# bacpop/ska.rust

Hardware: AMD Instinct MI355X
Metric: genomes/sec ska build+align, 1 000x5 Mbp k=31; bit-exact vs CPU (higher is better)
Workload: dtype u64

## Files before the change

ska.rust_amd/csrc/skx_api.cpp:

```cpp
#include "skx_internal.h"
#include "../../include/skx_host.h"
#include <algorithm>
#include <atomic>
#include <chrono>
#include <cmath>
#include <cstdarg>
#include <cstddef>
#include <cstdio>
#include <cstring>
#include <map>
#include <memory>
#include <mutex>
#include <numeric>
#include <optional>
#include <unordered_map>
#include <thread>
#include <cerrno>
#include <fcntl.h>
#include <sys/mman.h>
#include <sys/stat.h>
#include <unistd.h>

using namespace skx;

// ... 670 lines not shown
                std::vector<skx_key> nk; nk.reserve(kept);
                for (uint64_t i = 0; i < U; i++) if (hkeep[i] == 1) nk.push_back(a->host_keys[i]);
                a->host_keys.swap(nk);
            }
            a->n_kmers = kept;
        }
        SKX_HIP(hipStreamSynchronize(st));
        a->matrix = std::move(nm); a->present = std::move(p2); a->unambig = std::move(u2); a->mask = std::move(m2); a->vcount = std::move(v2);
        a->pitch = np; a->n_rows = kept;
        a->drop_lazy();
        a->stats_ready = true;
    }
    return SKX_OK;
}

extern "C" int skx_array_filter(skx_array *a, uint64_t min_count, int filter_ambig_as_missing, int filter_type, int mask_ambig,
                                int ignore_const_gaps, int update_kmers, int32_t *removed)
{
    return skx_guarded([&]() -> int {
    skx_ctx *ctx = a->ctx; hipStream_t st = ctx->stream;
    SKX_HIP(hipSetDevice(ctx->device));
    const uint64_t U = a->n_rows; const size_t S = a->names.size();
    ctx->cut_ranks = ctx->cut_blocks = 0;
    DevBuf<unsigned long long> tally;
    unsigned long long h_tally[2] = {0, 0};
    if (a->pieces && !a->stats_ready && !filter_ambig_as_missing && min_count >= 2 && a->total_samples == 0 && !knob("stats_eager"))
        SKX_TRY(pieces_stats_pass(a, min_count, &tally));
    else
        SKX_TRY(array_lazy_stats(a));
    DevBuf<uint8_t> keep; DevBuf<uint64_t> pos;
    SKX_TRY(keep.alloc(U)); SKX_TRY(pos.alloc(U + 1));
    uint64_t kept = 0, silent = 0;
    {
        StageTimer t(ctx, &ctx->tm.filter);
        FilterArgs fa{a->vcount.p, a->present.p, a->unambig.p, a->mask.p, U, (uint32_t)(a->total_samples ? a->total_samples : S), min_count, filter_ambig_as_missing, filter_type, ignore_const_gaps, keep.p};
        launch_filter_flags(fa, st);
        DevBuf<uint32_t> sc_sums; DevBuf<uint64_t> sc_offs;
        SKX_TRY(sc_sums.alloc(scan_u8_blocks(U))); SKX_TRY(sc_offs.alloc(scan_u8_blocks(U) + 1));
        launch_scan_u8(keep.p, pos.p, U, sc_sums.p, sc_offs.p, st);
        SKX_HIP(hipMemcpyAsync(&kept, pos.p + U, 8, hipMemcpyDeviceToHost, st));
        if (tally.p) SKX_HIP(hipMemcpyAsync(h_tally, tally.p, 16, hipMemcpyDeviceToHost, st));
// ... 380 lines not shown
```

ska.rust_amd/csrc/skx_append.hip:

```cpp
#include "skx_device.h"
#include <cstdlib>
#include <type_traits>

namespace skx {

typedef uint32_t u32x4 __attribute__((ext_vector_type(4)));
typedef const u32x4 __attribute__((address_space(1))) *g4_t;

#ifdef SKX_AP_PROF
__device__ unsigned long long g_ap_prof[16];
#define AP_PROF_START unsigned long long tprof = __builtin_readcyclecounter(), tacc[12] = {0, 0, 0, 0, 0, 0, 0, 0, 0, 0, 0, 0}
#define AP_PROF(i) do { const unsigned long long t_ = __builtin_readcyclecounter(); tacc[(i)] += t_ - tprof; tprof = t_; } while (0)
#define AP_PROF_FLUSH() do { for (int i_ = 0; i_ < 12; i_++) if (tacc[i_] && (i_ >= 6 || (threadIdx.x & 63) == 0)) atomicAdd(&g_ap_prof[i_], tacc[i_]); } while (0)
extern "C" void skx_debug_phase_prof(unsigned long long *out, int reset)
{
    unsigned long long h[16];
    (void)hipDeviceSynchronize();
    (void)hipMemcpyFromSymbol(h, HIP_SYMBOL(g_ap_prof), sizeof(h));
    for (int i = 0; i < 16; i++) out[i] = h[i];
    if (reset) { for (auto &x : h) x = 0; (void)hipMemcpyToSymbol(HIP_SYMBOL(g_ap_prof), h, sizeof(h)); }
}
#else
#define AP_PROF_START do { } while (0)
#define AP_PROF(i) do { } while (0)
// ... 501 lines not shown
        uint32_t rc = min_count ? cut : 0xFFFFFFFFu;
        if (ncnt && ncnt[j] > stage) rc = 0xFFFFFFFFu;
        r_cut[j] = rc;
        if (tally && nrank) pieces_cut_tally(nrank[j], rc, tally);
    }
}
void launch_pieces_cut(const uint16_t *plen, int n_samples, uint32_t cap, uint32_t min_count, const uint32_t *nrank, const uint32_t *ncnt, uint32_t stage, int n_blocks,
                       uint32_t *r_cut, unsigned long long *tally, hipStream_t st)
{
    if (n_blocks <= 0) return;
    hipLaunchKernelGGL(pieces_cut_kernel, dim3((unsigned)n_blocks), dim3(256), ((size_t)cap + 1) * 4, st, plen, n_samples, cap, min_count, nrank, ncnt, stage, r_cut, tally);
}

__global__ __launch_bounds__(256) void pieces_stats_kernel(const uint8_t *pieces, const uint16_t *plen, const uint16_t *perm, const uint32_t *nrank, const uint32_t *ncnt,
                                                           const uint64_t *roff, uint32_t cap, int S, uint32_t *o_present, uint32_t *o_unambig, uint32_t *o_mask,
                                                           uint32_t *o_vcount, int force_direct, uint32_t stage, uint32_t min_count, unsigned long long *tally)
{
    constexpr int W = 4;
    extern __shared__ __attribute__((aligned(16))) uint16_t s_stage[];
    const uint32_t PS_STAGE = stage;
    uint16_t *const s_pr = s_stage, *const s_un = s_stage + stage, *const s_mk = s_stage + 2 * (size_t)stage;
    const uint64_t j = blockIdx.x;
    const uint32_t nr = nrank[j], nrows = ncnt[j];
    const uint64_t r0 = roff[j];
    if (blockIdx.y * 256u * 8u * W >= nr && !(blockIdx.y == 0 && nrows)) return;
    const bool staged = gridDim.y == 1 && nrows <= PS_STAGE && !force_direct;
    const int lane = threadIdx.x & 63, wv = __builtin_amdgcn_readfirstlane((int)(threadIdx.x >> 6));
    const uint16_t *pl = plen + j * (uint64_t)S;
    uint32_t lim = nr;
    if (min_count && staged) {
        const uint32_t rc = pieces_cut_block(pl, S, cap, min_count, reinterpret_cast<uint32_t *>(s_stage));
        if (threadIdx.x == 0 && tally) pieces_cut_tally(nr, rc, tally);
        if (rc < lim) lim = rc;
    }
    const uint32_t nseen = (lim + 31u) / 32u * 32u < nr ? (lim + 31u) / 32u * 32u : nr;
    const uint32_t ncol = (lim + 31u) / 32u, ncg = ncol < 64u ? ncol : 64u;
    uint32_t G = 4, P = 1;
    if (staged && ncol) {
        G = (ncol + 63u) / 64u;
        for (P = 4u / G; P > 1u && (P / 2u) * G * 36u * 4u * ncg > PS_STAGE * 6u; P >>= 1) { }
    }
// ... 133 lines not shown
            const uint32_t r = rb + (uint32_t)src, prow = (uint32_t)__shfl((int)pp, src, 64);
            uint32_t m = 0;
            for (int t = lane; t < S; t += 64) {
                if ((uint32_t)pl[t] <= r) continue;
                const uint32_t x = *(reinterpret_cast<const uint32_t *>(pieces + (j * (uint64_t)S + t) * (cap / 2)) + (r >> 3));
                const uint32_t nib = (x >> ((r & 7u) * 4u)) & 15u;
                if (nib) m |= 1u << nib;
            }
#pragma unroll
            for (int dd = 32; dd >= 1; dd >>= 1) m |= __shfl_xor(m, dd, 64);
            if (lane == 0) { if (staged) s_mk[prow] = (uint16_t)m; else o_mask[r0 + prow] = m; }
        }
    }
    if (!staged) return;
    __syncthreads();
    for (uint32_t p = threadIdx.x; p < nrows; p += 256) {
        const uint32_t pr = s_pr[p];
        o_present[r0 + p] = pr; o_vcount[r0 + p] = pr;
        o_unambig[r0 + p] = s_un[p]; o_mask[r0 + p] = s_mk[p];
    }
}
namespace {
struct StatsLaunch { unsigned gy; int direct; uint32_t stage; bool bounded() const { return gy == 1 && !direct; } };
StatsLaunch stats_launch(uint32_t cap)
{
    static const int direct = knob("stats_direct") ? 1 : 0;
    return {(cap / 32 + 255u) / 256u, direct, (cap + 63u) / 64u * 64u};
}
}
void launch_pieces_stats(const uint8_t *pieces, const uint16_t *plen, const uint16_t *perm, const uint32_t *nrank, const uint32_t *ncnt, const uint64_t *roff, uint32_t cap,
                         int n_samples, int n_blocks, uint32_t *present, uint32_t *unambig, uint32_t *mask, uint32_t *vcount, hipStream_t st, uint32_t min_count, unsigned long long *tally)
{
    if (n_blocks <= 0) return;
    const StatsLaunch l = stats_launch(cap);
    if (!l.bounded()) min_count = 0;
    hipLaunchKernelGGL(pieces_stats_kernel, dim3((unsigned)n_blocks, l.gy), dim3(256), (size_t)l.stage * 6, st, pieces, plen, perm, nrank, ncnt, roff, cap, n_samples, present, unambig, mask, vcount,
                       l.direct, l.stage, min_count, tally);
}
uint32_t pieces_stats_bound(uint32_t cap) { const StatsLaunch l = stats_launch(cap); return l.bounded() ? l.stage : 0u; }
__global__ __launch_bounds__(256) void pieces_cells_kernel(const uint8_t *pieces, const uint16_t *plen, uint32_t cap, int S, unsigned long long *out)
{
    const uint64_t j = blockIdx.x;
    const int lane = threadIdx.x & 63;
    for (int s = blockIdx.y * 4 + (threadIdx.x >> 6); s < S; s += gridDim.y * 4) {
        const uint32_t pl = plen[j * (uint64_t)S + s];
        const uint32_t *src = reinterpret_cast<const uint32_t *>(pieces + (j * (uint64_t)S + s) * (cap / 2));
        uint32_t c = 0;
        for (uint32_t i = lane; i < (pl + 7u) / 8u; i += 64) { const uint32_t x = src[i]; uint32_t t = x | (x >> 1); t |= t >> 2; c += (uint32_t)__popc(t & 0x11111111u); }
#pragma unroll
        for (int dd = 32; dd >= 1; dd >>= 1) c += __shfl_xor(c, dd, 64);
        if (lane == 0 && c) atomicAdd(&out[s], (unsigned long long)c);
    }
// ... 29 lines not shown
    const uint32_t hi = __builtin_amdgcn_perm(0x4E42444Bu, 0x56535247u, idx);
    const uint32_t sel = ((m >> 3) & 0x01010101u) * 0xFFu;
    return (hi & sel) | (lo & ~sel);
}
template <bool KEPT>
__global__ __launch_bounds__(64 * PR_WAVES) void pieces_rows_kernel(PiecesRowsArgs a)
{
    extern __shared__ __attribute__((aligned(16))) unsigned char s_raw[];
    const uint32_t cap = a.cap;
    uint16_t *s_src = reinterpret_cast<uint16_t *>(s_raw);
    uint32_t *s_piece = reinterpret_cast<uint32_t *>(s_raw + (((size_t)cap + 16) * 2 + 15) / 16 * 16);
    const uint64_t j = (uint64_t)blockIdx.x + a.j_base;
    const uint32_t n = a.ncnt[j];
    if (n == 0) return;
    const uint64_t r0 = a.roff[j];
    const uint64_t k0 = KEPT ? a.kpos[r0] : 0;
    const uint32_t nout = KEPT ? (uint32_t)(a.kpos[r0 + n] - k0) : n;
    if (nout == 0) return;
    const int tid = threadIdx.x, lane = tid & 63, wv = tid >> 6;
    const uint64_t ocol = KEPT ? k0 : r0 - a.col_base;
    const uint32_t shift = (uint32_t)(ocol & 3u);
    const uint32_t ndw = (nout + shift + 3u) / 4u;
    const uint16_t *pj = a.perm + j * (uint64_t)cap;
    const uint32_t nr = a.nrank[j];
    const int S = a.n_samples;
    const int s_lo = blockIdx.y * a.samples_per_wg, s_hi = s_lo + a.samples_per_wg < S ? s_lo + a.samples_per_wg : S;
    uint32_t *pc = s_piece + (size_t)wv * (cap / 8 + 4);
    const unsigned char *pcb = reinterpret_cast<const unsigned char *>(pc);
    __shared__ uint32_t s_top;
    uint32_t nrw = (nr + 7u) / 8u;
    if (lane < 4) pc[cap / 8 + lane] = 0u;
    for (uint32_t t0 = 0; t0 < nout + shift; t0 += cap) {
        for (uint32_t i = tid; i < cap + 16u; i += blockDim.x) s_src[i] = (uint16_t)cap;
        if (KEPT && tid == 0) s_top = 0;
        __syncthreads();
        uint32_t top = 0;
        for (uint32_t r = tid; r < nr; r += blockDim.x) {
            const uint32_t p = pj[r];
            if (p == 0xFFFFu || p >= n) continue;
            uint32_t sc;
            if (!KEPT) sc = shift + p;
            else if (a.keep[r0 + p] == 1) sc = shift + (uint32_t)(a.kpos[r0 + p] - k0);
            else continue;
            if (sc >= t0 && sc < t0 + cap) { s_src[sc - t0] = (uint16_t)r; top = r + 1u; }
        }
        if (KEPT && top) atomicMax(&s_top, top);
        __syncthreads();
        if (KEPT && !a.full_pieces) nrw = (s_top + 7u) / 8u;
        const uint32_t v_lo = t0 / 4u, v_hi = (t0 + cap) / 4u < ndw ? (t0 + cap) / 4u : ndw;
        const int cnt = __builtin_amdgcn_readfirstlane(s_lo + wv < s_hi ? (s_hi - s_lo - wv + PR_WAVES - 1) / PR_WAVES : 0);
        const uint32_t n4 = (nrw + 3u) / 4u;
        const uint16_t *plj = a.plen + j * (uint64_t)S + s_lo + wv;
        uint4 *pc4 = reinterpret_cast<uint4 *>(pc);
        auto masked = [&](uint4 x, uint32_t i, uint32_t plw) {
            if (4u * i >= plw) x.x = 0u;
            if (4u * i + 1u >= plw) x.y = 0u;
// ... 46 lines not shown
            }
            __builtin_amdgcn_wave_barrier();
        }
        __syncthreads();
    }
}
void launch_pieces_rows(const PiecesRowsArgs &a, uint32_t n_blocks, hipStream_t st)
{
    if (!n_blocks || a.n_samples <= 0) return;
    PiecesRowsArgs b = a;
    int spw = a.n_samples;
    while (spw > PR_WAVES * 4 && (uint64_t)n_blocks * ((a.n_samples + spw - 1) / spw) < 8192) spw = (spw + 1) / 2;
    b.samples_per_wg = spw;
    const unsigned gy = (unsigned)((a.n_samples + spw - 1) / spw);
    const size_t lds = (((size_t)a.cap + 16) * 2 + 15) / 16 * 16 + (size_t)PR_WAVES * (a.cap / 8 + 4) * 4;
    if (a.keep) {
        (void)hipFuncSetAttribute((const void *)pieces_rows_kernel<true>, hipFuncAttributeMaxDynamicSharedMemorySize, (int)lds);
        hipLaunchKernelGGL(pieces_rows_kernel<true>, dim3(n_blocks, gy), dim3(64 * PR_WAVES), lds, st, b);
    } else {
        (void)hipFuncSetAttribute((const void *)pieces_rows_kernel<false>, hipFuncAttributeMaxDynamicSharedMemorySize, (int)lds);
        hipLaunchKernelGGL(pieces_rows_kernel<false>, dim3(n_blocks, gy), dim3(64 * PR_WAVES), lds, st, b);
    }
}

}

#include "skx_append_wide.inc"
```

ska.rust_amd/csrc/skx_device.h:

```cpp
#pragma once
#include <hip/hip_runtime.h>
#include <stdint.h>

namespace skx {

long knob(const char *name, long absent = 0);
int extract_tile_bases(int logB);
constexpr int MAX_LOGB = 13;
constexpr uint64_t EMPTY64 = ~0ull;

struct HashParams {
    int bits;
    int hb;
    uint32_t hmask;
    uint32_t c[4];
};
HashParams make_hash_params(int k);
__host__ __device__ inline uint32_t hround(uint32_t v, uint32_t c, int hb) { return (v * c) >> (32 - hb); }
__host__ __device__ inline void hmix_halves(uint32_t &L, uint32_t &R, const HashParams &p)
{
    L ^= hround(R, p.c[0], p.hb); R ^= hround(L, p.c[1], p.hb);
}
__host__ __device__ inline uint64_t hmix(uint64_t x, const HashParams &p)
{
// ... 120 lines not shown
    uint32_t nslots, cap;
    uint8_t *pieces; uint16_t *plen; uint16_t *perm; uint32_t *nrank;
    uint64_t *stage; uint32_t stride; uint32_t *ncnt;
    unsigned long long *probe;
    int *overflow;
    uint32_t rounds = 1;
    int *bar = nullptr;
};
bool append_ok(int bits, int logB, int logQ, uint32_t region_cap, uint32_t nslots, uint32_t cap);
void launch_append(const AppendArgs &a, uint32_t region_cap, hipStream_t st);
void launch_append_probe(const AppendArgs &a, uint32_t region_cap, unsigned blocks, hipStream_t st);
constexpr uint32_t APPEND_WIDE_MAX_CAP = 3072, APPEND_WIDE_MAX_SLOTS = 4096;
bool append_wide_ok(int bits, int logB, int logQ, uint32_t nslots, uint32_t cap);
void launch_append_wide(const AppendArgs &a, hipStream_t st);
void launch_append_wide_probe(const AppendArgs &a, unsigned blocks, hipStream_t st);
void launch_pieces_stats(const uint8_t *pieces, const uint16_t *plen, const uint16_t *perm, const uint32_t *nrank, const uint32_t *ncnt, const uint64_t *roff, uint32_t cap,
                         int n_samples, int n_blocks, uint32_t *present, uint32_t *unambig, uint32_t *mask, uint32_t *vcount, hipStream_t st, uint32_t min_count = 0, unsigned long long *tally = nullptr);
void launch_pieces_cut(const uint16_t *plen, int n_samples, uint32_t cap, uint32_t min_count, const uint32_t *nrank, const uint32_t *ncnt, uint32_t stage, int n_blocks,
                       uint32_t *r_cut, unsigned long long *tally, hipStream_t st);
uint32_t pieces_stats_bound(uint32_t cap);
void launch_pieces_cells(const uint8_t *pieces, const uint16_t *plen, uint32_t cap, int n_samples, int n_blocks, unsigned long long *out, hipStream_t st);
void launch_region_totals(const uint32_t *raw, int n_samples, int logB, unsigned long long *out, hipStream_t st);
struct PiecesRowsArgs {
    const uint8_t *pieces; const uint16_t *plen; const uint16_t *perm; const uint32_t *nrank; uint32_t cap; int n_samples;
    const uint32_t *ncnt; const uint64_t *roff;
    uint8_t *out; uint64_t pitch;
    uint32_t j_base = 0; uint64_t col_base = 0;
    const uint8_t *keep = nullptr; const uint64_t *kpos = nullptr;
    int mask_ambig = 0;
    int full_pieces = 0;
    int samples_per_wg = 0;
};
void launch_pieces_rows(const PiecesRowsArgs &a, uint32_t n_blocks, hipStream_t st);

void launch_gather_keys(const uint64_t *stage, uint32_t stride, const uint32_t *ncnt, const uint64_t *roff, int n_sub,
                        uint64_t *out, int unhash, HashParams hp, hipStream_t st);
void launch_hash_keys(const uint64_t *keys, uint64_t *words, uint64_t n, HashParams hp, hipStream_t st);
void launch_keys_cbor(const uint64_t *words, uint64_t n, HashParams hp, uint8_t *out, int *short_key, hipStream_t st);
void launch_unhash_dict(const uint64_t *words, uint64_t n, uint64_t *keys, uint8_t *bases, HashParams hp, hipStream_t st);

void launch_col_stats(const uint8_t *matrix, uint64_t pitch, int n_samples, uint64_t n_cols, uint32_t *present,
                      uint32_t *unambig, uint32_t *mask, int *bad_byte, hipStream_t st);
struct FilterArgs {
// ... 116 lines not shown
```

ska.rust_amd/csrc/skx_device.hip:

```cpp
#include "skx_device.h"
#include <cstdlib>

namespace skx {

HashParams make_hash_params(int k)
{
    HashParams p;
    p.bits = 2 * (k - 1);
    p.hb = k - 1;
    p.hmask = p.hb >= 32 ? ~0u : ((1u << p.hb) - 1);
    p.c[0] = 0x9E3779B1u; p.c[1] = 0x85EBCA6Bu; p.c[2] = 0xC2B2AE35u; p.c[3] = 0x27D4EB2Fu;
    return p;
}

__device__ static inline uint32_t revcomp_arm(uint32_t x, int n)
{
    x = __builtin_bitreverse32(x);
    x = ((x >> 1) & 0x55555555u) | ((x & 0x55555555u) << 1);
    x ^= 0xAAAAAAAAu;
    return n ? x >> (32 - 2 * n) : 0;
}

__device__ static inline void pack16(const uint32_t w[4], uint32_t &code, uint32_t &bad, uint32_t &nl)
{
// ... 1427 lines not shown
```

ska.rust_amd/csrc/skx_device2.inc:

```
namespace skx {

__device__ static inline uint32_t set_code(uint32_t b)
{
    switch (b) {
    case '-': return 0;
    case 'A': return 1;  case 'C': return 2;  case 'M': return 3;  case 'T': return 4;
    case 'W': return 5;  case 'Y': return 6;  case 'H': return 7;  case 'G': return 8;
    case 'R': return 9;  case 'S': return 10; case 'V': return 11; case 'K': return 12;
    case 'D': return 13; case 'B': return 14; case 'N': return 15;
    default: return 0xFF;
    }
}

__global__ __launch_bounds__(256) void col_stats_kernel(const uint8_t *matrix, uint64_t pitch, int n_samples, uint64_t n_cols,
                                                        uint32_t *present, uint32_t *unambig, uint32_t *mask, int *bad_byte)
{
    const uint64_t c0 = ((uint64_t)blockIdx.x * blockDim.x + threadIdx.x) * 4;
    if (c0 >= n_cols) return;
    uint32_t p[4] = {0, 0, 0, 0}, u[4] = {0, 0, 0, 0}, m[4] = {0, 0, 0, 0};
    int bad = 0;
    for (int s = 0; s < n_samples; s++) {
        const uint32_t x = *reinterpret_cast<const uint32_t *>(matrix + (uint64_t)s * pitch + c0);
#pragma unroll
        for (int i = 0; i < 4; i++) {
// ... 4 lines not shown
    }
#pragma unroll
    for (int i = 0; i < 4; i++)
        if (c0 + i < n_cols) { present[c0 + i] = p[i]; unambig[c0 + i] = u[i]; mask[c0 + i] = m[i]; }
    if (bad) *bad_byte = 1;
}
void launch_col_stats(const uint8_t *matrix, uint64_t pitch, int n_samples, uint64_t n_cols, uint32_t *present, uint32_t *unambig,
                      uint32_t *mask, int *bad_byte, hipStream_t st)
{
    if (!n_cols) return;
    uint64_t threads = (n_cols + 3) / 4;
    hipLaunchKernelGGL(col_stats_kernel, dim3((unsigned)((threads + 255) / 256)), dim3(256), 0, st, matrix, pitch, n_samples, n_cols,
                       present, unambig, mask, bad_byte);
}

__device__ static inline uint8_t filter_type_keep(int filter_type, int ignore_const_gaps, uint32_t m, bool has_gap)
{
    const uint32_t acgt = (1u << 1) | (1u << 2) | (1u << 4) | (1u << 8);
    switch (filter_type) {
    case 0: return 1;
    case 1: return (__popc(m) + ((has_gap && !ignore_const_gaps) ? 1 : 0)) > 1;
    case 2: return (m & ~acgt) == 0;
    default: return (__popc(m & acgt) + ((has_gap && !ignore_const_gaps) ? 1 : 0)) > 1;
    }
}
__global__ void filter_flags_kernel(FilterArgs a)
{
    const uint64_t c = (uint64_t)blockIdx.x * blockDim.x + threadIdx.x;
    if (c >= a.n_cols) return;
    const uint32_t present = a.present[c], unambig = a.unambig[c], m = a.mask[c];
    const uint32_t count = a.ambig_as_missing ? unambig : a.vcount[c];
    uint8_t keep;
    if (a.two_stage) {
        const bool has_gap = present < a.n_samples;
        if ((uint64_t)count < a.min_count) keep = 0;
        else keep = (__popc(m) + (has_gap ? 1 : 0)) > 1 ? 1 : 3;
    }
    else if (a.ambig_as_missing && count == 0) keep = 2;
    else if ((uint64_t)count < a.min_count) keep = 0;
    else keep = filter_type_keep(a.filter_type, a.ignore_const_gaps, m, present < a.n_samples);
    a.keep[c] = keep;
}
void launch_filter_flags(const FilterArgs &a, hipStream_t st)
{
    if (!a.n_cols) return;
    hipLaunchKernelGGL(filter_flags_kernel, dim3((unsigned)((a.n_cols + 255) / 256)), dim3(256), 0, st, a);
}

__device__ static inline uint8_t mask_ambig_byte(uint8_t b)
{
    return (b == 'A' || b == 'C' || b == 'G' || b == 'T' || b == 'U' || b == '-') ? b : (uint8_t)'N';
}
constexpr int CMP_ROWS = 4;
template <bool ORD = false>
__global__ __launch_bounds__(256) void compact_matrix_kernel(const uint8_t *in, uint64_t in_pitch, uint8_t *out, uint64_t out_pitch,
// ... 857 lines not shown
```

ska.rust_amd/csrc/skx_internal.h:

```cpp
#pragma once
#include "../../include/skx.h"
#include "skx_device.h"
#include <atomic>
#include <chrono>
#include <cstdio>
#include <condition_variable>
#include <functional>
#include <memory>
#include <mutex>
#include <new>
#include <thread>
#include <sys/types.h>
#include <stdexcept>
#include <string>
#include <vector>

namespace skx {

void set_error(const char *fmt, ...);

int hip_fail(hipError_t e, const char *what);

#define SKX_HIP(call) do { hipError_t e_ = (call); if (e_ != hipSuccess) return skx::hip_fail(e_, #call); } while (0)
#define SKX_TRY(call) do { int r_ = (call); if (r_ != SKX_OK) return r_; } while (0)
// ... 319 lines not shown
uint64_t nj_pitch(uint64_t S);
int nj_check_n(int n);
int nj_fits(skx_ctx *ctx, uint64_t S, uint64_t extra);
int nj_run_device(skx_ctx *ctx, DevBuf<double> &D, uint64_t pitch, uint32_t S, skx_nj_join *joins);
int planes_of_kept_rows(skx_array *a, const uint8_t *keep, int filt, DevBuf<uint64_t> &planes, uint64_t &wpr, uint64_t &rows, const int *order = nullptr);
void distance_filter_flags(skx_array *a, double min_freq, uint8_t *keep, hipStream_t st);
int cpu_budget();
int check_k(int k);
bool mappable_output_fd(int fd, off_t *pos);
int array_wide_words(skx_array *a, DevBuf<uint64_t> &tmp, const u128 **words);
int array_host_keys(skx_array *a, std::vector<skx_key> &hk);
int array_materialize(skx_array *a);
int array_lazy_stats(skx_array *a);
int array_lazy_window(skx_array *a, uint64_t r0, uint64_t nr, DevBuf<uint8_t> &buf, const uint8_t **win, uint64_t *wpitch);
int array_lazy_rows(skx_array *a, uint8_t *out, uint64_t pitch, uint32_t j_base = 0, uint32_t n_blocks = 0, uint64_t col_base = 0, const uint8_t *keep = nullptr,
                    const uint64_t *kpos = nullptr, int mask_ambig = 0, bool full_pieces = false);
int pieces_stats_pass(skx_array *a, uint64_t min_count, DevBuf<unsigned long long> *tally = nullptr);
int merge_batch(skx_ctx *ctx, skx_dictset *d, const char *const *names, skx_array **out);
inline uint64_t pitch_for(uint64_t cols) { return ((cols + 255) / 256) * 256 + 256; }
inline bool key_less(const skx_key &x, const skx_key &y) { return x.hi != y.hi ? x.hi < y.hi : x.lo < y.lo; }
inline bool key_eq(const skx_key &x, const skx_key &y) { return x.hi == y.hi && x.lo == y.lo; }
}
template <typename F>
inline int skx_guarded(F &&f) noexcept
{
    try { return f(); }
    catch (const std::bad_alloc &) { skx::set_error("out of host memory"); return SKX_ENOMEM; }
    catch (const std::exception &e) { skx::set_error("internal error: %s", e.what()); return SKX_EINVAL; }
    catch (...) { skx::set_error("internal error"); return SKX_EINVAL; }
}
```

ska.rust_amd/csrc/skx_merge.cpp:

```cpp
#include "skx_internal.h"
#include <algorithm>
#include <cmath>
#include <cstdlib>

using namespace skx;

extern "C" void skx_keyset_free(skx_keyset *ks) { delete ks; }
extern "C" int skx_keyset_size(const skx_keyset *ks, uint64_t *n) { *n = ks->total; return SKX_OK; }

static int keyset_finish(skx_keyset *ks)
{
    hipStream_t st = ks->ctx->stream;
    const uint64_t nsub = 1ull << ks->logN;
    SKX_TRY(ks->roff.alloc(nsub + 1));
    DevBuf<uint32_t> d_max; SKX_TRY(d_max.alloc(1));
    launch_scan_u32(ks->ncnt.p, ks->roff.p, nsub, d_max.p, st);
    SKX_HIP(hipMemcpyAsync(&ks->total, ks->roff.p + nsub, 8, hipMemcpyDeviceToHost, st));
    SKX_HIP(hipMemcpyAsync(&ks->max_rows, d_max.p, 4, hipMemcpyDeviceToHost, st));
    SKX_HIP(hipStreamSynchronize(st));
    if (getenv("SKX_DEBUG")) fprintf(stderr, "[skx] keyset: logN=%d sub-buckets=%llu rows=%llu mean=%.1f max=%u\n", ks->logN, (unsigned long long)nsub,
                                 (unsigned long long)ks->total, (double)ks->total / (double)nsub, ks->max_rows);
    return SKX_OK;
}

// ... 161 lines not shown
    aa.d = d->view(); aa.logN = rows->logN; aa.stage = rows->stage.p; aa.stride = rows->stride; aa.ncnt = rows->ncnt.p; aa.roff = rows->roff.p;
    aa.matrix = nullptr; aa.pitch = 0; aa.col_present = a->present.p; aa.col_unambig = a->unambig.p; aa.col_mask = a->mask.p;
    aa.max_rows = rows->max_rows; aa.missing = d_flag;
    return aa;
}
static int check_missing(skx_ctx *ctx, const int *d_flag)
{
    int missing = 0;
    SKX_HIP(hipMemcpyAsync(&missing, d_flag, 4, hipMemcpyDeviceToHost, ctx->stream));
    SKX_HIP(hipStreamSynchronize(ctx->stream));
    SKX_HIP(hipGetLastError());
    if (missing) { set_error("row keyset does not contain every split k-mer of the samples"); return SKX_EINVAL; }
    return SKX_OK;
}

int skx::pieces_stats_pass(skx_array *a, uint64_t min_count, DevBuf<unsigned long long> *tally)
{
    skx_ctx *ctx = a->ctx; hipStream_t st = ctx->stream;
    const skx_pieces *pc = a->pieces; const skx_keyset *blk = a->lazy_rows;
    const int S = (int)a->names.size(), nb = 1 << pc->logQ;
    if (!a->n_rows) return SKX_OK;
    const bool bounded = min_count >= 2 && tally && pieces_stats_bound(pc->cap);
    if (bounded) { SKX_TRY(tally->alloc(2)); SKX_TRY(tally->zero(st)); }
    {
        StageTimer t(ctx, &ctx->tm.assemble);
        KernelTimer kt(ctx, &ctx->tm.pieces_stats);
        launch_pieces_stats(pc->data.p, pc->plen.p, pc->perm.p, pc->nrank.p, blk->ncnt.p, blk->roff.p, pc->cap, S, nb, a->present.p, a->unambig.p, a->mask.p, a->vcount.p, st,
                            bounded ? (uint32_t)std::min<uint64_t>(min_count, 0xFFFFFFFEull) : 0u, bounded ? tally->p : nullptr);
    }
    if (!bounded) SKX_HIP(hipStreamSynchronize(st));
    SKX_HIP(hipGetLastError());
    return SKX_OK;
}

static int append_not_taken(skx_ctx *ctx, const char *why)
{
    ctx->merge_path = std::string("sorted: ") + why;
    if (getenv("SKX_DEBUG")) fprintf(stderr, "[skx] merge: %s\n", ctx->merge_path.c_str());
    return SKF_NOT_TAKEN;
}
static bool append_fits(bool wide, int bits, int logB, int lq, uint32_t region_cap, uint32_t nslots, uint32_t cap) { return wide ? append_wide_ok(bits, logB, lq, nslots, cap) : append_ok(bits, logB, lq, region_cap, nslots, cap); }
static uint32_t append_max_cap(bool wide) { return wide ? APPEND_WIDE_MAX_CAP : APPEND_MAX_CAP; }
static uint32_t append_max_slots(bool wide) { return wide ? APPEND_WIDE_MAX_SLOTS : APPEND_MAX_SLOTS; }
// ... 329 lines not shown
        a->stats_ready = true;
        return SKX_OK;
    }
    DevBuf<int> d_flag; SKX_TRY(d_flag.alloc(1)); SKX_TRY(d_flag.zero(st));
    if (a->n_rows) {
        AssembleArgs aa = assemble_args(a->lazy_dict, a->lazy_rows, a, d_flag.p);
        { StageTimer t(ctx, &ctx->tm.assemble); launch_assemble_lazy(a, aa, st, 1); }
        SKX_HIP(hipMemcpyAsync(a->vcount.p, a->present.p, a->n_rows * 4, hipMemcpyDeviceToDevice, st));
    }
    SKX_TRY(check_missing(ctx, d_flag.p));
    a->stats_ready = true;
    return SKX_OK;
}

int skx::array_lazy_rows(skx_array *a, uint8_t *out, uint64_t pitch, uint32_t j_base, uint32_t n_blocks, uint64_t col_base, const uint8_t *keep, const uint64_t *kpos,
                         int mask_ambig, bool full_pieces)
{
    skx_ctx *ctx = a->ctx; hipStream_t st = ctx->stream;
    if (a->pieces) {
        const skx_pieces *pc = a->pieces; const skx_keyset *rows = a->lazy_rows;
        PiecesRowsArgs pa{};
        pa.pieces = pc->data.p; pa.plen = pc->plen.p; pa.perm = pc->perm.p; pa.nrank = pc->nrank.p; pa.cap = pc->cap; pa.n_samples = (int)a->names.size();
        pa.ncnt = rows->ncnt.p; pa.roff = rows->roff.p;
        pa.out = out; pa.pitch = pitch; pa.j_base = j_base; pa.col_base = col_base;
        pa.keep = keep; pa.kpos = kpos; pa.mask_ambig = mask_ambig; pa.full_pieces = full_pieces ? 1 : 0;
        const uint32_t nb = n_blocks ? n_blocks : 1u << pc->logQ;
        if (keep) { KernelTimer kt(ctx, &ctx->tm.pieces_rows); launch_pieces_rows(pa, nb, st); }
        else { StageTimer t(ctx, &ctx->tm.assemble); launch_pieces_rows(pa, nb, st); }
        SKX_HIP(hipGetLastError());
        return SKX_OK;
    }
    DevBuf<int> d_flag; SKX_TRY(d_flag.alloc(1)); SKX_TRY(d_flag.zero(st));
    AssembleArgs aa = assemble_args(a->lazy_dict, a->lazy_rows, a, d_flag.p);
    aa.matrix = out; aa.pitch = pitch; aa.j_base = j_base; aa.col_base = col_base;
    aa.keep = keep; aa.kpos = kpos; aa.mask_ambig = mask_ambig;
    { StageTimer t(ctx, &ctx->tm.assemble); launch_assemble_lazy(a, aa, st, keep ? 2 : 0, n_blocks); }
    return check_missing(ctx, d_flag.p);
}
int skx::array_materialize(skx_array *a)
{
    if (!a->lazy()) return SKX_OK;
    skx_ctx *ctx = a->ctx; hipStream_t st = ctx->stream;
// ... 66 lines not shown
```

Baseline: 30770.

## Compute filter verdicts inside stats pass and compact kept rows per block

When the bounded pieces statistics pass applies, each block now evaluates the filter rule in LDS, ballots the verdicts, and writes per-block kept counts and 16-bit local output positions. A small single-block kernel scans the block counts into bases. The rows kernel then scatters matrix columns, per-row stats and device keys using these block-local positions. This replaces the separate flag kernel, full-length u8 scan and stats-compaction passes, and it shares the filter rule through a common header. In exchange it adds more code paths, a serial 1024-thread scan over all blocks, and a fallback for blocks that are not staged.

```diff
diff --git a/ska.rust_amd/csrc/skx_api.cpp b/ska.rust_amd/csrc/skx_api.cpp
--- a/ska.rust_amd/csrc/skx_api.cpp
+++ b/ska.rust_amd/csrc/skx_api.cpp
@@ -708,6 +708,53 @@
     return SKX_OK;
 }
 
+static int array_compact_by_block(skx_array *a, DevBuf<uint16_t> &kpos16, DevBuf<uint64_t> &kbase, DevBuf<uint8_t> &keep, uint64_t kept, int mask_ambig,
+                                  bool keys_follow)
+{
+    skx_ctx *ctx = a->ctx; hipStream_t st = ctx->stream;
+    const uint64_t U = a->n_rows; const size_t S = a->names.size();
+    if (kept == U && !mask_ambig) {
+        a->stats_ready = true;
+        SKX_HIP(hipStreamSynchronize(st));
+        return SKX_OK;
+    }
+    StageTimer t(ctx, &ctx->tm.compact);
+    const uint64_t np = pitch_for(kept);
+    DevBuf<uint8_t> nm; DevBuf<uint32_t> p2, u2, m2, v2; DevBuf<uint64_t> k2;
+    SKX_TRY(nm.alloc((uint64_t)S * np)); SKX_TRY(p2.alloc(kept)); SKX_TRY(u2.alloc(kept)); SKX_TRY(m2.alloc(kept)); SKX_TRY(v2.alloc(kept));
+    const bool move_keys = a->n_kmers == U && keys_follow;
+    const bool dev_keys = move_keys && (a->k <= 31 || a->host_keys.empty());
+    KeptByBlock kb;
+    kb.kbase = kbase.p; kb.kpos16 = kpos16.p;
+    kb.st_in[0] = a->present.p; kb.st_in[1] = a->unambig.p; kb.st_in[2] = a->mask.p; kb.st_in[3] = a->vcount.p;
+    kb.st_out[0] = p2.p; kb.st_out[1] = u2.p; kb.st_out[2] = m2.p; kb.st_out[3] = v2.p;
+    if (dev_keys) {
+        const int kw = a->k <= 31 ? 2 : 4;
+        SKX_TRY(k2.alloc(kept * (kw / 2)));
+        kb.key_in = reinterpret_cast<const uint32_t *>(a->keys.p); kb.key_out = reinterpret_cast<uint32_t *>(k2.p); kb.key_words = kw;
+    }
+    SKX_TRY(array_lazy_rows(a, nm.p, np, 0, 0, 0, nullptr, nullptr, mask_ambig, false, &kb));
+    if (mask_ambig) launch_mask_ambig_stats(m2.p, kept, st);
+    if (move_keys) {
+        if (dev_keys) a->keys = std::move(k2);
+        else {
+            std::vector<uint8_t> hkeep(U);
+            SKX_HIP(hipMemcpyAsync(hkeep.data(), keep.p, U, hipMemcpyDeviceToHost, st));
+            SKX_HIP(hipStreamSynchronize(st));
+            std::vector<skx_key> nk; nk.reserve(kept);
+            for (uint64_t i = 0; i < U; i++) if (hkeep[i] == 1) nk.push_back(a->host_keys[i]);
+            a->host_keys.swap(nk);
+        }
+        a->n_kmers = kept;
+    }
+    SKX_HIP(hipStreamSynchronize(st));
+    a->matrix = std::move(nm); a->present = std::move(p2); a->unambig = std::move(u2); a->mask = std::move(m2); a->vcount = std::move(v2);
+    a->pitch = np; a->n_rows = kept;
+    a->drop_lazy();
+    a->stats_ready = true;
+    return SKX_OK;
+}
+
 extern "C" int skx_array_filter(skx_array *a, uint64_t min_count, int filter_ambig_as_missing, int filter_type, int mask_ambig,
                                 int ignore_const_gaps, int update_kmers, int32_t *removed)
 {
@@ -718,7 +765,35 @@
     ctx->cut_ranks = ctx->cut_blocks = 0;
     DevBuf<unsigned long long> tally;
     unsigned long long h_tally[2] = {0, 0};
-    if (a->pieces && !a->stats_ready && !filter_ambig_as_missing && min_count >= 2 && a->total_samples == 0 && !knob("stats_eager"))
+    const bool bounded = a->pieces && !a->stats_ready && !filter_ambig_as_missing && min_count >= 2 && a->total_samples == 0 && !knob("stats_eager");
+    const bool by_block = bounded && U && pieces_stats_bound(a->pieces->cap) && a->pieces->cap <= 8192 && !knob("filter_generic");
+    if (getenv("SKX_DEBUG")) fprintf(stderr, "[skx] filter chain: %s\n", by_block ? "verdicts from the bounded statistics pass, kept rows by block" : "flags, scan, compaction");
+    if (by_block) {
+        const uint32_t nb = 1u << a->pieces->logQ;
+        DevBuf<uint16_t> kpos16; DevBuf<uint32_t> blk_kept; DevBuf<uint64_t> kbase; DevBuf<uint8_t> keep;
+        SKX_TRY(kpos16.alloc(U)); SKX_TRY(blk_kept.alloc(nb)); SKX_TRY(kbase.alloc((uint64_t)nb + 1));
+        const bool keys_follow = update_kmers != 0;
+        if (keys_follow && a->n_kmers == U && a->k > 31 && !a->host_keys.empty()) SKX_TRY(keep.alloc(U));
+        StatsVerdict fv;
+        fv.kpos16 = kpos16.p; fv.blk_kept = blk_kept.p; fv.keep = keep.p; fv.n_samples = (uint32_t)S; fv.min_count = min_count;
+        fv.filter_type = filter_type; fv.ignore_const_gaps = ignore_const_gaps;
+        SKX_TRY(pieces_stats_pass(a, min_count, &tally, &fv));
+        uint64_t kept = 0;
+        {
+            StageTimer t(ctx, &ctx->tm.filter);
+            launch_block_bases(blk_kept.p, nb, kbase.p, st);
+            SKX_HIP(hipMemcpyAsync(&kept, kbase.p + nb, 8, hipMemcpyDeviceToHost, st));
+            SKX_HIP(hipMemcpyAsync(h_tally, tally.p, 16, hipMemcpyDeviceToHost, st));
+            SKX_HIP(hipStreamSynchronize(st));
+        }
+        ctx->cut_ranks = h_tally[0]; ctx->cut_blocks = h_tally[1];
+        if (getenv("SKX_DEBUG")) fprintf(stderr, "[skx] filter: min_count %llu, the rank bound left %llu ranks unread over %llu of %d row blocks\n", (unsigned long long)min_count, h_tally[0], h_tally[1], 1 << a->pieces->logQ);
+        SKX_TRY(array_compact_by_block(a, kpos16, kbase, keep, kept, mask_ambig, keys_follow));
+        SKX_HIP(hipGetLastError());
+        if (removed) *removed = (int32_t)(U - kept);
+        return SKX_OK;
+    }
+    if (bounded)
         SKX_TRY(pieces_stats_pass(a, min_count, &tally));
     else
         SKX_TRY(array_lazy_stats(a));
diff --git a/ska.rust_amd/csrc/skx_append.hip b/ska.rust_amd/csrc/skx_append.hip
--- a/ska.rust_amd/csrc/skx_append.hip
+++ b/ska.rust_amd/csrc/skx_append.hip
@@ -1,4 +1,5 @@
 #include "skx_device.h"
+#include "skx_filter_rule.h"
 #include <cstdlib>
 #include <type_traits>
 
@@ -539,7 +540,8 @@
 
 __global__ __launch_bounds__(256) void pieces_stats_kernel(const uint8_t *pieces, const uint16_t *plen, const uint16_t *perm, const uint32_t *nrank, const uint32_t *ncnt,
                                                            const uint64_t *roff, uint32_t cap, int S, uint32_t *o_present, uint32_t *o_unambig, uint32_t *o_mask,
-                                                           uint32_t *o_vcount, int force_direct, uint32_t stage, uint32_t min_count, unsigned long long *tally)
+                                                           uint32_t *o_vcount, int force_direct, uint32_t stage, uint32_t min_count, unsigned long long *tally,
+                                                           StatsVerdict fv)
 {
     constexpr int W = 4;
     extern __shared__ __attribute__((aligned(16))) uint16_t s_stage[];
@@ -548,8 +550,9 @@
     const uint64_t j = blockIdx.x;
     const uint32_t nr = nrank[j], nrows = ncnt[j];
     const uint64_t r0 = roff[j];
+    const bool staged = gridDim.y == 1 && nrows <= PS_STAGE && !force_direct;
+    if (fv.kpos16 && blockIdx.y == 0 && threadIdx.x == 0 && (!nrows || !staged)) fv.blk_kept[j] = 0;
     if (blockIdx.y * 256u * 8u * W >= nr && !(blockIdx.y == 0 && nrows)) return;
-    const bool staged = gridDim.y == 1 && nrows <= PS_STAGE && !force_direct;
     const int lane = threadIdx.x & 63, wv = __builtin_amdgcn_readfirstlane((int)(threadIdx.x >> 6));
     const uint16_t *pl = plen + j * (uint64_t)S;
     uint32_t lim = nr;
@@ -713,10 +716,41 @@
     }
     if (!staged) return;
     __syncthreads();
+    __shared__ unsigned long long s_vbits[128];
+    __shared__ uint32_t s_vbase[128];
+    if (fv.kpos16) {
+        const uint32_t nw = (nrows + 63u) / 64u;
+        for (uint32_t base = 0; base < nrows; base += 256) {
+            const uint32_t p = base + threadIdx.x;
+            bool k = false;
+            if (p < nrows) {
+                const uint32_t pr = s_pr[p];
+                k = filter_row_verdict(pr, s_un[p], s_mk[p], pr, fv.n_samples, fv.min_count, 0, fv.filter_type, fv.ignore_const_gaps) == 1;
+            }
+            const unsigned long long b = __ballot(k);
+            if (lane == 0 && (base >> 6) + (uint32_t)wv < nw) s_vbits[(base >> 6) + (uint32_t)wv] = b;
+        }
+        __syncthreads();
+        if (wv == 0) {
+            const uint32_t w0 = 2u * (uint32_t)lane, c0 = w0 < nw ? (uint32_t)__popcll(s_vbits[w0]) : 0u, c1 = w0 + 1u < nw ? (uint32_t)__popcll(s_vbits[w0 + 1u]) : 0u;
+            uint32_t incl = c0 + c1;
+#pragma unroll
+            for (int dd = 1; dd < 64; dd <<= 1) { const uint32_t o = (uint32_t)__shfl_up((int)incl, dd, 64); if (lane >= dd) incl += o; }
+            s_vbase[w0] = incl - c0 - c1; s_vbase[w0 + 1u] = incl - c1;
+            if (lane == 63) fv.blk_kept[j] = incl;
+        }
+        __syncthreads();
+    }
     for (uint32_t p = threadIdx.x; p < nrows; p += 256) {
         const uint32_t pr = s_pr[p];
         o_present[r0 + p] = pr; o_vcount[r0 + p] = pr;
         o_unambig[r0 + p] = s_un[p]; o_mask[r0 + p] = s_mk[p];
+        if (fv.kpos16) {
+            const unsigned long long w = s_vbits[p >> 6];
+            const uint32_t k = (uint32_t)(w >> (p & 63u)) & 1u;
+            fv.kpos16[r0 + p] = k ? (uint16_t)(s_vbase[p >> 6] + (uint32_t)__popcll(w & ((1ull << (p & 63u)) - 1ull))) : (uint16_t)0xFFFFu;
+            if (fv.keep) fv.keep[r0 + p] = (uint8_t)k;
+        }
     }
 }
 namespace {
@@ -728,13 +762,44 @@
 }
 }
 void launch_pieces_stats(const uint8_t *pieces, const uint16_t *plen, const uint16_t *perm, const uint32_t *nrank, const uint32_t *ncnt, const uint64_t *roff, uint32_t cap,
-                         int n_samples, int n_blocks, uint32_t *present, uint32_t *unambig, uint32_t *mask, uint32_t *vcount, hipStream_t st, uint32_t min_count, unsigned long long *tally)
+                         int n_samples, int n_blocks, uint32_t *present, uint32_t *unambig, uint32_t *mask, uint32_t *vcount, hipStream_t st, uint32_t min_count, unsigned long long *tally,
+                         const StatsVerdict *verdict)
 {
     if (n_blocks <= 0) return;
     const StatsLaunch l = stats_launch(cap);
     if (!l.bounded()) min_count = 0;
+    StatsVerdict fv;
+    if (verdict && min_count) fv = *verdict;
     hipLaunchKernelGGL(pieces_stats_kernel, dim3((unsigned)n_blocks, l.gy), dim3(256), (size_t)l.stage * 6, st, pieces, plen, perm, nrank, ncnt, roff, cap, n_samples, present, unambig, mask, vcount,
-                       l.direct, l.stage, min_count, tally);
+                       l.direct, l.stage, min_count, tally, fv);
+}
+__global__ __launch_bounds__(1024) void block_bases_kernel(const uint32_t *blk_kept, uint32_t n_blocks, uint64_t *kbase)
+{
+    __shared__ uint32_t s_wave[16];
+    __shared__ unsigned long long s_run;
+    const uint32_t tid = threadIdx.x, lane = tid & 63u, wv = tid >> 6;
+    if (tid == 0) s_run = 0;
+    __syncthreads();
+    for (uint32_t b0 = 0; b0 < n_blocks; b0 += 1024) {
+        const uint32_t own = b0 + tid < n_blocks ? blk_kept[b0 + tid] : 0u;
+        uint32_t incl = own;
+#pragma unroll
+        for (int dd = 1; dd < 64; dd <<= 1) { const uint32_t o = (uint32_t)__shfl_up((int)incl, dd, 64); if (lane >= (uint32_t)dd) incl += o; }
+        if (lane == 63) s_wave[wv] = incl;
+        __syncthreads();
+        uint32_t before = 0, all = 0;
+        for (uint32_t w = 0; w < 16; w++) { const uint32_t t = s_wave[w]; if (w < wv) before += t; all += t; }
+        const unsigned long long run = s_run;
+        if (b0 + tid < n_blocks) kbase[b0 + tid] = run + before + (incl - own);
+        __syncthreads();
+        if (tid == 0) s_run = run + all;
+        __syncthreads();
+    }
+    if (tid == 0) kbase[n_blocks] = s_run;
+}
+void launch_block_bases(const uint32_t *blk_kept, uint32_t n_blocks, uint64_t *kbase, hipStream_t st)
+{
+    hipLaunchKernelGGL(block_bases_kernel, dim3(1), dim3(1024), 0, st, blk_kept, n_blocks, kbase);
 }
 uint32_t pieces_stats_bound(uint32_t cap) { const StatsLaunch l = stats_launch(cap); return l.bounded() ? l.stage : 0u; }
 __global__ __launch_bounds__(256) void pieces_cells_kernel(const uint8_t *pieces, const uint16_t *plen, uint32_t cap, int S, unsigned long long *out)
@@ -794,10 +859,22 @@
     const uint32_t n = a.ncnt[j];
     if (n == 0) return;
     const uint64_t r0 = a.roff[j];
-    const uint64_t k0 = KEPT ? a.kpos[r0] : 0;
-    const uint32_t nout = KEPT ? (uint32_t)(a.kpos[r0 + n] - k0) : n;
+    const bool by_block = KEPT && a.kb.kpos16 != nullptr;
+    const uint64_t k0 = KEPT ? (by_block ? a.kb.kbase[j] : a.kpos[r0]) : 0;
+    const uint32_t nout = KEPT ? (uint32_t)((by_block ? a.kb.kbase[j + 1] : a.kpos[r0 + n]) - k0) : n;
     if (nout == 0) return;
     const int tid = threadIdx.x, lane = tid & 63, wv = tid >> 6;
+    if (by_block && blockIdx.y == 0 && a.kb.st_out[0]) {
+        for (uint32_t p = tid; p < n; p += blockDim.x) {
+            const uint32_t q = a.kb.kpos16[r0 + p];
+            if (q == 0xFFFFu) continue;
+            const uint64_t o = k0 + q;
+#pragma unroll
+            for (int i = 0; i < 4; i++) a.kb.st_out[i][o] = a.kb.st_in[i][r0 + p];
+            if (a.kb.key_words == 2) reinterpret_cast<uint2 *>(a.kb.key_out)[o] = reinterpret_cast<const uint2 *>(a.kb.key_in)[r0 + p];
+            else if (a.kb.key_words == 4) reinterpret_cast<uint4 *>(a.kb.key_out)[o] = reinterpret_cast<const uint4 *>(a.kb.key_in)[r0 + p];
+        }
+    }
     const uint64_t ocol = KEPT ? k0 : r0 - a.col_base;
     const uint32_t shift = (uint32_t)(ocol & 3u);
     const uint32_t ndw = (nout + shift + 3u) / 4u;
@@ -820,6 +897,7 @@
             if (p == 0xFFFFu || p >= n) continue;
             uint32_t sc;
             if (!KEPT) sc = shift + p;
+            else if (by_block) { const uint32_t q = a.kb.kpos16[r0 + p]; if (q == 0xFFFFu) continue; sc = shift + q; }
             else if (a.keep[r0 + p] == 1) sc = shift + (uint32_t)(a.kpos[r0 + p] - k0);
             else continue;
             if (sc >= t0 && sc < t0 + cap) { s_src[sc - t0] = (uint16_t)r; top = r + 1u; }
@@ -896,7 +974,7 @@
     b.samples_per_wg = spw;
     const unsigned gy = (unsigned)((a.n_samples + spw - 1) / spw);
     const size_t lds = (((size_t)a.cap + 16) * 2 + 15) / 16 * 16 + (size_t)PR_WAVES * (a.cap / 8 + 4) * 4;
-    if (a.keep) {
+    if (a.keep || a.kb.kpos16) {
         (void)hipFuncSetAttribute((const void *)pieces_rows_kernel<true>, hipFuncAttributeMaxDynamicSharedMemorySize, (int)lds);
         hipLaunchKernelGGL(pieces_rows_kernel<true>, dim3(n_blocks, gy), dim3(64 * PR_WAVES), lds, st, b);
     } else {
diff --git a/ska.rust_amd/csrc/skx_device.h b/ska.rust_amd/csrc/skx_device.h
--- a/ska.rust_amd/csrc/skx_device.h
+++ b/ska.rust_amd/csrc/skx_device.h
@@ -158,19 +158,31 @@
 bool append_wide_ok(int bits, int logB, int logQ, uint32_t nslots, uint32_t cap);
 void launch_append_wide(const AppendArgs &a, hipStream_t st);
 void launch_append_wide_probe(const AppendArgs &a, unsigned blocks, hipStream_t st);
+struct StatsVerdict {
+    uint16_t *kpos16 = nullptr; uint32_t *blk_kept = nullptr; uint8_t *keep = nullptr;
+    uint32_t n_samples = 0; uint64_t min_count = 0; int filter_type = 0, ignore_const_gaps = 0;
+};
 void launch_pieces_stats(const uint8_t *pieces, const uint16_t *plen, const uint16_t *perm, const uint32_t *nrank, const uint32_t *ncnt, const uint64_t *roff, uint32_t cap,
-                         int n_samples, int n_blocks, uint32_t *present, uint32_t *unambig, uint32_t *mask, uint32_t *vcount, hipStream_t st, uint32_t min_count = 0, unsigned long long *tally = nullptr);
+                         int n_samples, int n_blocks, uint32_t *present, uint32_t *unambig, uint32_t *mask, uint32_t *vcount, hipStream_t st, uint32_t min_count = 0, unsigned long long *tally = nullptr,
+                         const StatsVerdict *verdict = nullptr);
+void launch_block_bases(const uint32_t *blk_kept, uint32_t n_blocks, uint64_t *kbase, hipStream_t st);
 void launch_pieces_cut(const uint16_t *plen, int n_samples, uint32_t cap, uint32_t min_count, const uint32_t *nrank, const uint32_t *ncnt, uint32_t stage, int n_blocks,
                        uint32_t *r_cut, unsigned long long *tally, hipStream_t st);
 uint32_t pieces_stats_bound(uint32_t cap);
 void launch_pieces_cells(const uint8_t *pieces, const uint16_t *plen, uint32_t cap, int n_samples, int n_blocks, unsigned long long *out, hipStream_t st);
 void launch_region_totals(const uint32_t *raw, int n_samples, int logB, unsigned long long *out, hipStream_t st);
+struct KeptByBlock {
+    const uint64_t *kbase = nullptr; const uint16_t *kpos16 = nullptr;
+    const uint32_t *st_in[4] = {nullptr, nullptr, nullptr, nullptr}; uint32_t *st_out[4] = {nullptr, nullptr, nullptr, nullptr};
+    const uint32_t *key_in = nullptr; uint32_t *key_out = nullptr; int key_words = 0;
+};
 struct PiecesRowsArgs {
     const uint8_t *pieces; const uint16_t *plen; const uint16_t *perm; const uint32_t *nrank; uint32_t cap; int n_samples;
     const uint32_t *ncnt; const uint64_t *roff;
     uint8_t *out; uint64_t pitch;
     uint32_t j_base = 0; uint64_t col_base = 0;
     const uint8_t *keep = nullptr; const uint64_t *kpos = nullptr;
+    KeptByBlock kb;
     int mask_ambig = 0;
     int full_pieces = 0;
     int samples_per_wg = 0;
diff --git a/ska.rust_amd/csrc/skx_device.hip b/ska.rust_amd/csrc/skx_device.hip
--- a/ska.rust_amd/csrc/skx_device.hip
+++ b/ska.rust_amd/csrc/skx_device.hip
@@ -1,4 +1,5 @@
 #include "skx_device.h"
+#include "skx_filter_rule.h"
 #include <cstdlib>
 
 namespace skx {
diff --git a/ska.rust_amd/csrc/skx_device2.inc b/ska.rust_amd/csrc/skx_device2.inc
--- a/ska.rust_amd/csrc/skx_device2.inc
+++ b/ska.rust_amd/csrc/skx_device2.inc
@@ -42,31 +42,19 @@
                        present, unambig, mask, bad_byte);
 }
 
-__device__ static inline uint8_t filter_type_keep(int filter_type, int ignore_const_gaps, uint32_t m, bool has_gap)
-{
-    const uint32_t acgt = (1u << 1) | (1u << 2) | (1u << 4) | (1u << 8);
-    switch (filter_type) {
-    case 0: return 1;
-    case 1: return (__popc(m) + ((has_gap && !ignore_const_gaps) ? 1 : 0)) > 1;
-    case 2: return (m & ~acgt) == 0;
-    default: return (__popc(m & acgt) + ((has_gap && !ignore_const_gaps) ? 1 : 0)) > 1;
-    }
-}
 __global__ void filter_flags_kernel(FilterArgs a)
 {
     const uint64_t c = (uint64_t)blockIdx.x * blockDim.x + threadIdx.x;
     if (c >= a.n_cols) return;
     const uint32_t present = a.present[c], unambig = a.unambig[c], m = a.mask[c];
-    const uint32_t count = a.ambig_as_missing ? unambig : a.vcount[c];
+    const uint32_t vcount = a.ambig_as_missing ? unambig : a.vcount[c];
     uint8_t keep;
     if (a.two_stage) {
         const bool has_gap = present < a.n_samples;
-        if ((uint64_t)count < a.min_count) keep = 0;
+        if ((uint64_t)vcount < a.min_count) keep = 0;
         else keep = (__popc(m) + (has_gap ? 1 : 0)) > 1 ? 1 : 3;
     }
-    else if (a.ambig_as_missing && count == 0) keep = 2;
-    else if ((uint64_t)count < a.min_count) keep = 0;
-    else keep = filter_type_keep(a.filter_type, a.ignore_const_gaps, m, present < a.n_samples);
+    else keep = filter_row_verdict(present, unambig, m, vcount, a.n_samples, a.min_count, a.ambig_as_missing, a.filter_type, a.ignore_const_gaps);
     a.keep[c] = keep;
 }
 void launch_filter_flags(const FilterArgs &a, hipStream_t st)
diff --git a/ska.rust_amd/csrc/skx_filter_rule.h b/ska.rust_amd/csrc/skx_filter_rule.h
--- /dev/null
+++ b/ska.rust_amd/csrc/skx_filter_rule.h
@@ -0,0 +1,29 @@
+#pragma once
+#include <stdint.h>
+#if defined(__HIPCC__)
+#define SKX_HD __host__ __device__
+#else
+#define SKX_HD
+#endif
+namespace skx {
+
+SKX_HD static inline uint8_t filter_type_keep(int filter_type, int ignore_const_gaps, uint32_t m, bool has_gap)
+{
+    const uint32_t acgt = (1u << 1) | (1u << 2) | (1u << 4) | (1u << 8);
+    switch (filter_type) {
+    case 0: return 1;
+    case 1: return (__builtin_popcount(m) + ((has_gap && !ignore_const_gaps) ? 1 : 0)) > 1;
+    case 2: return (m & ~acgt) == 0;
+    default: return (__builtin_popcount(m & acgt) + ((has_gap && !ignore_const_gaps) ? 1 : 0)) > 1;
+    }
+}
+SKX_HD static inline uint8_t filter_row_verdict(uint32_t present, uint32_t unambig, uint32_t m, uint32_t vcount, uint32_t n_samples, uint64_t min_count,
+                                                int ambig_as_missing, int filter_type, int ignore_const_gaps)
+{
+    const uint32_t count = ambig_as_missing ? unambig : vcount;
+    if (ambig_as_missing && count == 0) return 2;
+    if ((uint64_t)count < min_count) return 0;
+    return filter_type_keep(filter_type, ignore_const_gaps, m, present < n_samples);
+}
+
+}
diff --git a/ska.rust_amd/csrc/skx_internal.h b/ska.rust_amd/csrc/skx_internal.h
--- a/ska.rust_amd/csrc/skx_internal.h
+++ b/ska.rust_amd/csrc/skx_internal.h
@@ -357,8 +357,8 @@
 int array_lazy_stats(skx_array *a);
 int array_lazy_window(skx_array *a, uint64_t r0, uint64_t nr, DevBuf<uint8_t> &buf, const uint8_t **win, uint64_t *wpitch);
 int array_lazy_rows(skx_array *a, uint8_t *out, uint64_t pitch, uint32_t j_base = 0, uint32_t n_blocks = 0, uint64_t col_base = 0, const uint8_t *keep = nullptr,
-                    const uint64_t *kpos = nullptr, int mask_ambig = 0, bool full_pieces = false);
-int pieces_stats_pass(skx_array *a, uint64_t min_count, DevBuf<unsigned long long> *tally = nullptr);
+                    const uint64_t *kpos = nullptr, int mask_ambig = 0, bool full_pieces = false, const KeptByBlock *by_block = nullptr);
+int pieces_stats_pass(skx_array *a, uint64_t min_count, DevBuf<unsigned long long> *tally = nullptr, const StatsVerdict *verdict = nullptr);
 int merge_batch(skx_ctx *ctx, skx_dictset *d, const char *const *names, skx_array **out);
 inline uint64_t pitch_for(uint64_t cols) { return ((cols + 255) / 256) * 256 + 256; }
 inline bool key_less(const skx_key &x, const skx_key &y) { return x.hi != y.hi ? x.hi < y.hi : x.lo < y.lo; }
diff --git a/ska.rust_amd/csrc/skx_merge.cpp b/ska.rust_amd/csrc/skx_merge.cpp
--- a/ska.rust_amd/csrc/skx_merge.cpp
+++ b/ska.rust_amd/csrc/skx_merge.cpp
@@ -199,7 +199,7 @@
     return SKX_OK;
 }
 
-int skx::pieces_stats_pass(skx_array *a, uint64_t min_count, DevBuf<unsigned long long> *tally)
+int skx::pieces_stats_pass(skx_array *a, uint64_t min_count, DevBuf<unsigned long long> *tally, const StatsVerdict *verdict)
 {
     skx_ctx *ctx = a->ctx; hipStream_t st = ctx->stream;
     const skx_pieces *pc = a->pieces; const skx_keyset *blk = a->lazy_rows;
@@ -211,7 +211,7 @@
         StageTimer t(ctx, &ctx->tm.assemble);
         KernelTimer kt(ctx, &ctx->tm.pieces_stats);
         launch_pieces_stats(pc->data.p, pc->plen.p, pc->perm.p, pc->nrank.p, blk->ncnt.p, blk->roff.p, pc->cap, S, nb, a->present.p, a->unambig.p, a->mask.p, a->vcount.p, st,
-                            bounded ? (uint32_t)std::min<uint64_t>(min_count, 0xFFFFFFFEull) : 0u, bounded ? tally->p : nullptr);
+                            bounded ? (uint32_t)std::min<uint64_t>(min_count, 0xFFFFFFFEull) : 0u, bounded ? tally->p : nullptr, bounded ? verdict : nullptr);
     }
     if (!bounded) SKX_HIP(hipStreamSynchronize(st));
     SKX_HIP(hipGetLastError());
@@ -571,7 +571,7 @@
 }
 
 int skx::array_lazy_rows(skx_array *a, uint8_t *out, uint64_t pitch, uint32_t j_base, uint32_t n_blocks, uint64_t col_base, const uint8_t *keep, const uint64_t *kpos,
-                         int mask_ambig, bool full_pieces)
+                         int mask_ambig, bool full_pieces, const KeptByBlock *by_block)
 {
     skx_ctx *ctx = a->ctx; hipStream_t st = ctx->stream;
     if (a->pieces) {
@@ -581,8 +581,9 @@
         pa.ncnt = rows->ncnt.p; pa.roff = rows->roff.p;
         pa.out = out; pa.pitch = pitch; pa.j_base = j_base; pa.col_base = col_base;
         pa.keep = keep; pa.kpos = kpos; pa.mask_ambig = mask_ambig; pa.full_pieces = full_pieces ? 1 : 0;
+        if (by_block) pa.kb = *by_block;
         const uint32_t nb = n_blocks ? n_blocks : 1u << pc->logQ;
-        if (keep) { KernelTimer kt(ctx, &ctx->tm.pieces_rows); launch_pieces_rows(pa, nb, st); }
+        if (keep || by_block) { KernelTimer kt(ctx, &ctx->tm.pieces_rows); launch_pieces_rows(pa, nb, st); }
         else { StageTimer t(ctx, &ctx->tm.assemble); launch_pieces_rows(pa, nb, st); }
         SKX_HIP(hipGetLastError());
         return SKX_OK;
```

Result: no change. 31020, median of 4 (+0.8%).
